# tarepan/DDSP-SVC-official

Hardware: AMD Instinct MI355X
Metric: audio samples/sec @44.1kHz CombSub synth (higher is better)
Workload: dtype f32 storage and accumulation; products of the GEMM / FIR contractions split-bf16x3 (hi*hi+hi*lo+lo*hi), of the attention split-bf16 from three pieces (6 products) for the feature projections and two (3 products) for the context sums; everything else f32; `value_fp32_mfma` is the leg with every produ; 1 GPU; CombSub 44.1 kHz, batch=64x2 s per GPU (Fr=172, T=88064), units/f0/volume/spk_id -> audio, seeded random weights, in-kernel noise

## Files before the change

### ddsp-svc-official_amd/csrc/gemm_f32.h

```cpp
#pragma once
#include "common.h"
#include "gemm_group.h"

#include <stdlib.h>
#include <type_traits>

namespace gemm {

enum { A_PLAIN = 0, A_CONV3 = 1, A_FRAMES = 2, A_CONVK = 3, A_DWCONV = 4 };

struct Args {
    const float* A;
    const float* B;
    int M, N, K;
    int64_t lda, ldb;
    int zdiv;
    int64_t sA_hi, sA_lo, sB_hi, sB_lo;
    int Fr, Cin;
    int tap_shift;
    int ktaps, dil;
    float in_slope;
    const float* zeros;
    int sub_from, parent_tn;
    int math;
    const float* B_split;
    int A_split;
    int xcd;
    int xcd_cut;
    int kz;
};

constexpr int BK = 32;
typedef float f32x4_u __attribute__((ext_vector_type(4), aligned(4)));

template <class E, class = void>
struct epi_wants_pair : std::false_type {};
template <class E>
struct epi_wants_pair<E, std::void_t<decltype(E::kPair)>> : std::true_type {};
template <class E, class = void>
struct epi_has_store4 : std::false_type {};
template <class E>
struct epi_has_store4<E, std::void_t<decltype(E::kStore4)>> : std::true_type {};
// ... 971 lines not shown
```

### ddsp-svc-official_amd/csrc/gemm_ln.h

```cpp
#pragma once
#include "gemm_f32.h"

#include <atomic>
#include <stdlib.h>

namespace gemm {

struct LnArgs {
    const float* A;
    const float* W;
    int64_t lda, ldw;
    int M, K;
    const float* bias;
    const float* res;
    float* X;
    const float* gamma;
    const float* beta;
    float* Y;
    int y_split;
    int Fr = 1, Cin = 32, tap_shift = 0;
    const float* zeros = nullptr;
    const float* dw_taps = nullptr;
    const float* dw_bias = nullptr;
    const int* n_frames = nullptr;
    int dw_left = 15;
};

struct PreResidual {
    struct State {
        f32x4 res[2][4];
        f32x4 bias4[4];
    };
    template <int RB>
    __device__ __forceinline__ void load(State& s, const LnArgs& g, int m0, int rg0, int lr, int cg, int lh) const {
#pragma unroll
        for (int b = 0; b < RB; ++b) {
            const int row_m = m0 + 32 * (rg0 + b) + lr;
#pragma unroll
            for (int q = 0; q < 4; ++q) {
                s.res[b][q] = f32x4{0.f, 0.f, 0.f, 0.f};
                if (row_m < g.M) s.res[b][q] = *(const f32x4*)(g.res + (int64_t)row_m * 256 + 32 * cg + 8 * q + 4 * lh);
            }
        }
#pragma unroll
        for (int q = 0; q < 4; ++q) s.bias4[q] = *(const f32x4*)(g.bias + 32 * cg + 8 * q + 4 * lh);
    }
    __device__ __forceinline__ f32x4 apply(const State& s, const LnArgs&, int b, int q, int, int, f32x4 acc) const {
        f32x4 v;
#pragma unroll
        for (int e = 0; e < 4; ++e) v[e] = s.res[b][q][e] + (acc[e] + s.bias4[q][e]);
        return v;
    }
};

constexpr int LN_BM = 64, LN_N = 256, LN_NS = 4;
constexpr int LN_STAGE = (LN_BM + LN_N) * 32;
constexpr size_t LN_LDS_BYTES = (size_t)LN_NS * LN_STAGE * sizeof(float);

constexpr int DWF_K = 31, DWF_C = 64, DWF_ROWS = LN_BM + DWF_K - 1, DWF_NSW = 3;
constexpr int DWF_W = LN_N * 32, DWF_IMG = LN_BM * 32;
constexpr int DWF_AIMG = DWF_NSW * DWF_W, DWF_RAW = DWF_AIMG + 4 * DWF_IMG, DWF_TAPS = DWF_RAW + 96 * DWF_C;
static_assert(DWF_TAPS + 32 * DWF_C == LN_NS * LN_STAGE, "the A_DWCONV layout fills the same LDS");

template <int NS, int RB, bool ASPLIT, int A_MODE, class Pre>
__global__ void __launch_bounds__(1024 / RB) kernel_res_ln(LnArgs g, Pre pre) {
    extern __shared__ __attribute__((aligned(1024))) float ln_lds[];
    float* const lds = ln_lds;
    constexpr int NWAVE = 16 / RB;
    const int tid = threadIdx.x, lane = tid & 63, wave = __builtin_amdgcn_readfirstlane(tid >> 6);
    const int rg0 = RB == 1 ? wave >> 3 : 0, cg = wave & 7, lr = lane & 31, lh = lane >> 5;
    const int nk = g.K / 32;
    int m0 = blockIdx.x * LN_BM;
    int dw_b = 0, dw_f0 = 0;
    if constexpr (A_MODE == A_DWCONV) {
        const int ftiles = (g.Fr + LN_BM - 1) / LN_BM;
        dw_b = blockIdx.x / ftiles;
        dw_f0 = (blockIdx.x % ftiles) * LN_BM;
        m0 = dw_b * g.Fr + dw_f0;
        g.M = dw_b * g.Fr + (dw_f0 + LN_BM < g.Fr ? dw_f0 + LN_BM : g.Fr);
    }

    typename Pre::State pst;
    pre.template load<RB>(pst, g, m0, rg0, lr, cg, lh);
    f32x4 gam4[4], bet4[4];
#pragma unroll
    for (int q = 0; q < 4; ++q) {
        const int c0 = 32 * cg + 8 * q + 4 * lh;
        gam4[q] = *(const f32x4*)(g.gamma + c0);
        bet4[q] = *(const f32x4*)(g.beta + c0);
    }
    static_assert(A_MODE == A_PLAIN || ((A_MODE == A_CONV3 || A_MODE == A_DWCONV) && RB == 2), "conv modes: eight waves, one A piece each");
    static_assert(A_MODE != A_DWCONV || ASPLIT, "the convolved operand is written in the split layout");

    typedef __bf16 bf16x8 __attribute__((ext_vector_type(8)));
    f32x16 acc[RB];
#pragma unroll
    for (int b = 0; b < RB; ++b)
#pragma unroll
        for (int r = 0; r < 16; ++r) acc[b][r] = 0.f;
    auto products = [&](const float* ast, const float* wst) {
        f32x4 xv[RB][4], wv[4];
#pragma unroll
        for (int b = 0; b < RB; ++b) {
            const int row = 32 * (rg0 + b) + lr;
            const float* rp = ast + row * 32;
#pragma unroll
            for (int c = 0; c < 4; ++c) xv[b][c] = *(const f32x4*)(rp + 4 * ((4 * lh + c) ^ ((row >> 1) & 7)));
        }
        {
            const int row = 32 * cg + lr;
            const float* rp = wst + row * 32;
#pragma unroll
            for (int c = 0; c < 4; ++c) wv[c] = *(const f32x4*)(rp + 4 * ((4 * lh + c) ^ ((row >> 1) & 7)));
        }
#pragma unroll
        for (int half = 0; half < 2; ++half) {
            const bf16x8 wh = __builtin_bit_cast(bf16x8, wv[2 * half]), wl = __builtin_bit_cast(bf16x8, wv[2 * half + 1]);
#pragma unroll
            for (int b = 0; b < RB; ++b) {
                bf16x8 xh, xl;
                if constexpr (ASPLIT) {
                    xh = __builtin_bit_cast(bf16x8, xv[b][2 * half]);
                    xl = __builtin_bit_cast(bf16x8, xv[b][2 * half + 1]);
                } else {
                    typedef float f32x2p __attribute__((ext_vector_type(2)));
                    typedef __bf16 bf16x2p __attribute__((ext_vector_type(2)));
                    ddsp_u32x4 wh_, wl_;
#pragma unroll
                    for (int d = 0; d < 4; ++d) {
                        const f32x4& src = d < 2 ? xv[b][2 * half] : xv[b][2 * half + 1];
                        f32x2p r = {src[(2 * d) & 3], src[(2 * d + 1) & 3]};
                        const uint32_t hh = __builtin_bit_cast(uint32_t, __builtin_convertvector(r, bf16x2p));
                        wh_[d] = hh;
                        r = r - (f32x2p){__builtin_bit_cast(float, hh << 16), __builtin_bit_cast(float, hh & 0xffff0000u)};
                        wl_[d] = __builtin_bit_cast(uint32_t, __builtin_convertvector(r, bf16x2p));
                    }
                    xh = __builtin_bit_cast(bf16x8, wh_);
                    xl = __builtin_bit_cast(bf16x8, wl_);
                }
                acc[b] = __builtin_amdgcn_mfma_f32_32x32x16_bf16(wh, xl, acc[b], 0, 0, 0);
                acc[b] = __builtin_amdgcn_mfma_f32_32x32x16_bf16(wl, xh, acc[b], 0, 0, 0);
                acc[b] = __builtin_amdgcn_mfma_f32_32x32x16_bf16(wh, xh, acc[b], 0, 0, 0);
            }
        }
    };

    if constexpr (A_MODE == A_DWCONV) {
        typedef float f32x2d __attribute__((ext_vector_type(2)));
        typedef __bf16 bf16x2d __attribute__((ext_vector_type(2)));
        float* const aimg = lds + DWF_AIMG;
        float* const raw = lds + DWF_RAW;
        float* const taps = lds + DWF_TAPS;
        const int nb = nk / 2;
        const int n_in = ddsp_row_frames(g.n_frames, dw_b, g.Fr);
        const int c4 = lane & 15;
        const float* rsrc[3];
        int radv[3];
#pragma unroll
        for (int i = 0; i < 3; ++i) {
            const int r = (wave + 8 * i) * 4 + (lane >> 4);
            const int f = dw_f0 + r - g.dw_left;
            const bool ok = r < DWF_ROWS && f >= 0 && f < n_in;
            rsrc[i] = ok ? g.A + ((int64_t)dw_b * g.Fr + f) * g.lda + 4 * c4 : g.zeros + 4 * c4;
            radv[i] = ok ? DWF_C : 0;
        }
        const int trow = 4 * wave + (lane >> 4);
        const float* const tsrc = trow < DWF_K ? g.dw_taps + (int64_t)trow * g.K + 4 * c4 : g.dw_bias + 4 * c4;
        const float* wsrc[4];
#pragma unroll
        for (int i = 0; i < 4; ++i) {
            const int n = (wave + 8 * i) * 8 + (lane >> 3);
            wsrc[i] = g.W + (int64_t)n * g.ldw + 4 * ((lane & 7) ^ ((n >> 1) & 7));
        }
        auto dma = [&](const float* p, float* dst) {
            __builtin_amdgcn_global_load_lds((const __attribute__((address_space(1))) void*)p,
                                             (__attribute__((address_space(3))) void*)dst, 16, 0, 0);
        };
        auto issue_raw = [&](int j) {
#pragma unroll
            for (int i = 0; i < 3; ++i) dma(rsrc[i] + j * radv[i], raw + (wave + 8 * i) * 256);
// ... 187 lines not shown
        for (int q = 0; q < 4; ++q) {
            const int c0 = 32 * cg + 8 * q + 4 * lh;
            f32x4 o;
#pragma unroll
            for (int e = 0; e < 4; ++e) o[e] = fmaf(d[b][q][e] * rs, gam4[q][e], bet4[q][e]);
            if (g.y_split) {
                const ddsp_u32x4 pk = ddsp_split4_pair(o, lh != 0, 32);
                if (row_ok) *(ddsp_u32x4*)(g.Y + (int64_t)row_m * LN_N + c0) = pk;
            } else if (row_ok)
                *(f32x4*)(g.Y + (int64_t)row_m * LN_N + c0) = o;
        }
    }
}

inline bool res_ln_ok(const LnArgs& g) {
    return g.K % 32 == 0 && g.K >= 64 && g.lda % 4 == 0 && g.ldw % 4 == 0 && g.M >= 1 &&
           (((uintptr_t)g.A | (uintptr_t)g.W | (uintptr_t)g.bias | (uintptr_t)g.res | (uintptr_t)g.X | (uintptr_t)g.gamma |
             (uintptr_t)g.beta | (uintptr_t)g.Y) % 16) == 0;
}

template <int RB, bool ASPLIT, int A_MODE = A_PLAIN, class Pre = PreResidual>
inline hipError_t launch_res_ln_rb(hipStream_t st, const LnArgs& g, const Pre& pre = Pre{}) {
    static std::atomic<uint64_t> done{0};
    int dev = 0;
    hipError_t e = hipGetDevice(&dev);
    if (e != hipSuccess) return e;
    const uint64_t bit = 1ull << (dev & 63);
    auto kfn = kernel_res_ln<LN_NS, RB, ASPLIT, A_MODE, Pre>;
    if (!(done.load(std::memory_order_acquire) & bit)) {
        e = hipFuncSetAttribute((const void*)kfn, hipFuncAttributeMaxDynamicSharedMemorySize, (int)LN_LDS_BYTES);
        if (e != hipSuccess) return e;
        done.fetch_or(bit, std::memory_order_release);
    }
    const int64_t tiles = A_MODE == A_DWCONV ? (int64_t)(g.M / g.Fr) * ((g.Fr + LN_BM - 1) / LN_BM) : (g.M + LN_BM - 1) / LN_BM;
    hipLaunchKernelGGL(kfn, dim3((unsigned)tiles), dim3(1024 / RB), LN_LDS_BYTES, st, g, pre);
    return hipSuccess;
}
inline hipError_t launch_res_ln(hipStream_t st, const LnArgs& g, bool a_split = true) {
    return a_split ? launch_res_ln_rb<2, true>(st, g) : launch_res_ln_rb<2, false>(st, g);
}

inline bool res_ln_dwconv_ok(const LnArgs& g) {
    return res_ln_ok(g) && g.K % 64 == 0 && g.Fr >= 1 && g.M % g.Fr == 0 && g.zeros && g.dw_taps && g.dw_bias && g.dw_left >= 0 &&
           g.dw_left < DWF_K && (((uintptr_t)g.zeros | (uintptr_t)g.dw_taps | (uintptr_t)g.dw_bias) % 16) == 0;
}
inline bool res_ln_dwconv_fills(int64_t B, int64_t Fr) {
    const int64_t own = B * ((Fr + LN_BM - 1) / LN_BM), rows = (B * Fr + LN_BM - 1) / LN_BM;
    return B >= 1 && Fr >= 1 && 4 * own <= 5 * rows;
}
inline hipError_t launch_res_ln_dwconv(hipStream_t st, const LnArgs& g) { return launch_res_ln_rb<2, true, A_DWCONV>(st, g); }

}
```

### ddsp-svc-official_amd/csrc/unit2ctrl_fwd.hip

```cpp
#include "gemm_f32.h"
#include "gemm_ws.h"
#include "gemm_ln.h"
#include "performer_attn.h"
#include "u2c.h"

using namespace u2c;

namespace {

__device__ __forceinline__ void store_group8(float* __restrict__ dst, const float (&x)[8], bool split) {
    if (split) {
        ddsp_u32x4 hi, lo;
        ddsp_split8(x, hi, lo);
        *(ddsp_u32x4*)dst = hi;
        *(ddsp_u32x4*)(dst + 4) = lo;
    } else {
        *(f32x4*)dst = f32x4{x[0], x[1], x[2], x[3]};
        *(f32x4*)(dst + 4) = f32x4{x[4], x[5], x[6], x[7]};
    }
}

__device__ __forceinline__ void pack_conv3_body(const float* __restrict__ w, int Cout, int Cin, float* __restrict__ out,
                                                int vb, int vgrid, bool split) {
    const int64_t groups = (int64_t)Cout * 3 * (Cin / 8);
// ... 325 lines not shown
            const int64_t id = spk_id[n_spk_id == 1 ? 0 : m / Fr];
            if (id >= 1 && id <= w.n_spk) {
                const v4 e = *(const v4*)(w.spk_table + (id - 1) * D + n);
#pragma unroll
                for (int j = 0; j < 4; ++j) v[j] += e[j];
            } else {
                __hip_atomic_store(err, DDSP_DEV_ERR_SPK_ID, __ATOMIC_RELAXED, __HIP_MEMORY_SCOPE_SYSTEM);
            }
        }
        return v;
    }
};

struct PreEmbed {
    EpiEmbed e;
    struct State {};
    template <int RB>
    __device__ __forceinline__ void load(State&, const gemm::LnArgs&, int, int, int, int, int) const {}
    __device__ __forceinline__ f32x4 apply(const State&, const gemm::LnArgs&, int, int, int m, int c0, f32x4 acc) const {
        return e.embed4(m, c0, acc);
    }
};

struct LnPending {
    const float* part;
    const float* bias;
    float* x_out;
    int has_res;
};
constexpr int KS_SPLITS = 4;
constexpr int KS_MAX_ROWS = 256;
constexpr int64_t U2C_PRESPLIT_MIN_ROWS = 8192;
constexpr int64_t U2C_DWCONV_FUSE_MIN_ROWS = 10240;
constexpr int64_t ATTN_BF16_MIN = 256;
__global__ void __launch_bounds__(256) layernorm_kernel(const float* __restrict__ x, const float* __restrict__ gamma,
                                                        const float* __restrict__ beta, int64_t rows,
                                                        float* __restrict__ out, int split, LnPending pend = LnPending{nullptr, nullptr, nullptr, 0}) {
    const int lane = threadIdx.x & 63;
    const int64_t m = (int64_t)blockIdx.x * 4 + (threadIdx.x >> 6);
    if (m >= rows) return;
    f32x4 v;
    if (pend.part) {
        const f32x4 p0 = *(const f32x4*)(pend.part + m * D + lane * 4), p1 = *(const f32x4*)(pend.part + (rows + m) * D + lane * 4);
        const f32x4 p2 = *(const f32x4*)(pend.part + (2 * rows + m) * D + lane * 4), p3 = *(const f32x4*)(pend.part + (3 * rows + m) * D + lane * 4);
        v = (p0 + p1) + (p2 + p3);
        if (pend.bias) v = v + *(const f32x4*)(pend.bias + lane * 4);
        if (pend.has_res) v = *(const f32x4*)(x + m * D + lane * 4) + v;
        *(f32x4*)(pend.x_out + m * D + lane * 4) = v;
    } else {
        v = *(const f32x4*)(x + m * D + lane * 4);
    }
    const float mean = wave_sum((v[0] + v[1]) + (v[2] + v[3])) * (1.0f / D);
    f32x4 d;
    float ss = 0.f;
#pragma unroll
    for (int j = 0; j < 4; ++j) {
        d[j] = v[j] - mean;
        ss = fmaf(d[j], d[j], ss);
    }
    const float rstd = 1.0f / sqrtf(wave_sum(ss) * (1.0f / D) + 1e-5f);
    const f32x4 ga = *(const f32x4*)(gamma + lane * 4), be = *(const f32x4*)(beta + lane * 4);
    f32x4 o;
#pragma unroll
    for (int j = 0; j < 4; ++j) o[j] = fmaf(d[j] * rstd, ga[j], be[j]);
    if (split)
        *(ddsp_u32x4*)(out + m * D + lane * 4) = ddsp_split4_pair(o, (lane & 1) != 0, 1);
// ... 426 lines not shown
        g.math = lin_math;
        if (presplit_w) {
            g.B = packed;
            g.B_split = packed;
            g.A_split = a_is_split;
        }
    };
    static const bool dw_tiled = [] { const char* e = getenv("DDSP_DW_PAIR"); return !(e && e[0] == '1'); }();
    bool conv_split = false;
    {
        gemm::Args g = gemm::make(in.units, w.n_unit, bf.w1, 3 * w.n_unit, iM, D, 3 * w.n_unit);
        set_b(g, bf.w1, 0);
        g.tap_shift = w.causal ? -1 : 0;
        g.Fr = (int)Fr;
        g.Cin = w.n_unit;
        g.zeros = zero_page;
        conv_split = ksplit && gemm::dma_ok(g) && g.K % (32 * KS_SPLITS) == 0 && w.n_unit % 32 == 0 && (3 * D) % (32 * KS_SPLITS) == 0 &&
                     w.n_unit + 32 <= DDSP_ZERO_FLOATS;
        if (conv_split) {
            g.K /= KS_SPLITS;
            g.kz = g.K;
            gemm::EpiStore e{bf.kpart, D, nullptr, 1, M * D, 0};
            PROF(PF_U2C_GEMM_CONV3, 2.0 * M * D * 3 * w.n_unit, 4.0 * M * (w.n_unit + D),
                 (gemm::dma_go<64, 64, gemm::EpiStore, 4, 4, gemm::A_CONV3>(st, g, KS_SPLITS, e)));
        } else {
            gemm::EpiStore e{bf.t1, D, w.prenet_conv1_b, 1, 0, 0};
            PROF(PF_U2C_GEMM_CONV3, 2.0 * M * D * 3 * w.n_unit, 4.0 * M * (w.n_unit + D),
                 (gemm::launch<true, true, gemm::A_CONV3>(st, g, 1, e)));
        }
    }
    PROF(PF_U2C_ROWWISE, 0, 4.0 * M * D,
         hipLaunchKernelGGL(groupnorm_stats_kernel, dim3(4, (unsigned)B), dim3(64 * GN_LANES), 0, st, bf.t1, (int)Fr, bf.gst,
                            conv_split ? bf.kpart : nullptr, w.prenet_conv1_b, M, in.n_frames));
    PROF(PF_U2C_ROWWISE, 0, 8.0 * M * D,
         hipLaunchKernelGGL(groupnorm_lrelu_kernel, dim3(grid_for(M * (D / 4))), dim3(256), 0, st, bf.t1, bf.gst,
                            w.prenet_gn_w, w.prenet_gn_b, M, (int)Fr, bf.t2, asplit, in.n_frames));
    float* x = bf.l[0].x_in;
    {
        gemm::Args g = gemm::make(bf.t2, D, bf.w2, 3 * D, iM, D, 3 * D);
        set_b(g, bf.w2, asplit);
        g.tap_shift = w.causal ? -1 : 0;
        g.Fr = (int)Fr;
        g.Cin = D;
        g.zeros = zero_page;
        if (conv_split) {
            g.K /= KS_SPLITS;
            g.kz = g.K;
            EpiEmbed e{bf.kpart, w.prenet_conv2_b, in.f0, in.phase, in.volume, w, in.spk_id, in.n_spk_id, in.mix, (int)Fr, dev_err, M * D};
            PROF(PF_U2C_GEMM_CONV3, 2.0 * M * D * 3 * D, 8.0 * M * D,
                 (gemm::dma_go<64, 64, EpiEmbed, 4, 4, gemm::A_CONV3>(st, g, KS_SPLITS, e)));
            pending = LnPending{bf.kpart, nullptr, x, 0};
        } else {
            EpiEmbed e{x, w.prenet_conv2_b, in.f0, in.phase, in.volume, w, in.spk_id, in.n_spk_id, in.mix, (int)Fr, dev_err, 0};
            gemm::LnArgs la = ln_args(g, x, x, w.prenet_conv2_b, w.layer[0].norm_w, w.layer[0].norm_b, bf.l[0].y);
            la.Fr = (int)Fr;
            la.Cin = D;
            la.tap_shift = g.tap_shift;
            la.zeros = zero_page;
            if (ln_fusable(g, la) && g.A_split && D + 32 <= DDSP_ZERO_FLOATS) {
                PROF(PF_U2C_GEMM_CONV3, 2.0 * M * D * 3 * D, 12.0 * M * D,
                     DDSP_HIP(ctx, (gemm::launch_res_ln_rb<2, true, gemm::A_CONV3, PreEmbed>(st, la, PreEmbed{e}))));
                ln_done = true;
            } else
                PROF(PF_U2C_GEMM_CONV3, 2.0 * M * D * 3 * D, 8.0 * M * D, (gemm::launch<true, true, gemm::A_CONV3>(st, g, 1, e)));
        }
    }
    DDSP_LAUNCH_CHECK(ctx);

    const unsigned rows_g = (unsigned)ceil_div64(M, 4), rows8_g = (unsigned)ceil_div64(M8, 4);
    auto feature_maps = [&](const LayerBufs& b, const float* proj) {
        gemm::Args g = gemm::make(b.q, DH, proj, DH, (int)M8, NF, DH);
// ... 270 lines not shown
extern "C" int ddsp_u2c_dwconv_pw2(ddsp_ctx* ctx, void* stream, const float* glu, const float* taps, const float* dw_bias,
                                   const float* W_split, const float* bias, const float* res, const float* gamma,
                                   const float* beta, const int* n_frames, int B, int Fr, int causal, int fused, float* scratch,
                                   float* X, float* Y) {
    DDSP_REQUIRE(ctx, ctx && glu && taps && dw_bias && W_split && bias && res && gamma && beta && X && Y && (fused || scratch),
                 "ddsp_u2c_dwconv_pw2: null argument");
    DDSP_REQUIRE(ctx, B >= 1 && Fr >= 1 && (int64_t)B * Fr < (1 << 26), "ddsp_u2c_dwconv_pw2: bad shape");
    const float* zero_page = nullptr;
    if (int rc = ddsp_zero_page(ctx, &zero_page)) return rc;
    hipStream_t st = (hipStream_t)stream;
    const int M = B * Fr, left = causal ? DWK - 1 : DWK / 2;
    gemm::LnArgs a{fused ? glu : scratch, W_split, INNER, INNER, M, INNER, bias, res, X, gamma, beta, Y, 1};
    a.Fr = Fr;
    a.zeros = zero_page;
    a.dw_taps = taps;
    a.dw_bias = dw_bias;
    a.n_frames = n_frames;
    a.dw_left = left;
    DDSP_REQUIRE(ctx, gemm::res_ln_dwconv_ok(a) && ((uintptr_t)glu % 16) == 0, "ddsp_u2c_dwconv_pw2: 16-byte aligned operands");
    DDSP_ENTER_DEVICE(ctx);
    ddsp_prof_begin(ctx, st, PF_OTHER);
    if (fused) {
        DDSP_HIP(ctx, gemm::launch_res_ln_dwconv(st, a));
    } else {
        hipLaunchKernelGGL(dwconv_tile_kernel, dim3(INNER / DWT_C, (unsigned)(B * ((Fr + DWT_F - 1) / DWT_F))), dim3(256), 0, st, glu,
                           taps, dw_bias, B, Fr, scratch, left, 1, n_frames);
        DDSP_HIP(ctx, gemm::launch_res_ln(st, a, true));
    }
    ddsp_prof_end(ctx, st, 2.0 * M * (double)D * INNER + 2.0 * M * (double)INNER * DWK, 4.0 * M * (INNER + 4.0 * D));
    DDSP_LAUNCH_CHECK(ctx);
    return DDSP_OK;
}

extern "C" int ddsp_unit2ctrl_fwd(ddsp_ctx* ctx, void* stream, const ddsp_u2c_weights* wp, const float* units,
                                  const float* f0_frames, const float* phase_frames, const float* volume,
                                  const int64_t* spk_id, int64_t n_spk_id, const int64_t* mix_ids_host,
                                  const float* mix_w_host, int n_mix, int64_t B, int64_t Fr, const int32_t* n_frames,
                                  float* ctrl) {
    return unit2ctrl_fwd_any(ctx, stream, wp, units, f0_frames, phase_frames, volume, spk_id, n_spk_id, mix_ids_host, mix_w_host,
                             n_mix, B, Fr, n_frames, ctrl);
}

extern "C" int ddsp_unit2ctrl_fwd_rowmix(ddsp_ctx* ctx, void* stream, const ddsp_u2c_weights* wp, const float* units,
                                         const float* f0_frames, const float* phase_frames, const float* volume,
                                         const int32_t* mix_ids_dev, const float* mix_w_dev, int K, int64_t B, int64_t Fr,
                                         const int32_t* n_frames, float* ctrl) {
    DDSP_REQUIRE(ctx, ctx && mix_ids_dev && mix_w_dev, "ddsp_unit2ctrl_fwd_rowmix: null mix table");
    DDSP_REQUIRE(ctx, K >= 1 && K <= 16, "ddsp_unit2ctrl_fwd_rowmix: 1 <= K <= 16 mixed speakers per row");
    const int64_t one_id = 1;
    const float zero_w = 0.f;
    return unit2ctrl_fwd_any(ctx, stream, wp, units, f0_frames, phase_frames, volume, nullptr, 0, &one_id, &zero_w, 1, B, Fr,
                             n_frames, ctrl, mix_ids_dev, mix_w_dev, K);
}

extern "C" int ddsp_unit2ctrl_fwd_framemix(ddsp_ctx* ctx, void* stream, const ddsp_u2c_weights* wp, const float* units,
                                           const float* f0_frames, const float* phase_frames, const float* volume,
                                           const int32_t* mix_ids_dev, const float* mix_w_dev, int K, int64_t B, int64_t Fr,
                                           const int32_t* n_frames, float* ctrl) {
    DDSP_REQUIRE(ctx, ctx && mix_ids_dev && mix_w_dev, "ddsp_unit2ctrl_fwd_framemix: null mix table");
    DDSP_REQUIRE(ctx, K >= 1 && K <= 16, "ddsp_unit2ctrl_fwd_framemix: 1 <= K <= 16 mixed speakers per frame");
    const int64_t one_id = 1;
    const float zero_w = 0.f;
    return unit2ctrl_fwd_any(ctx, stream, wp, units, f0_frames, phase_frames, volume, nullptr, 0, &one_id, &zero_w, 1, B, Fr,
                             n_frames, ctrl, mix_ids_dev, mix_w_dev, K, 1);
}

// ... 29 lines not shown
```

### ddsp-svc-official_amd/hipddsp/__init__.py

```python
import ctypes
import math as _math
import numbers
import os
import threading

import torch

_HERE = os.path.dirname(os.path.abspath(__file__))
LIB_PATH = os.path.join(_HERE, "libddsp_amd.so")

DDSP_OK, DDSP_ERR_ARG, DDSP_ERR_HIP, DDSP_ERR_OOM = 0, -1, -2, -3

COMB_NONE, COMB_SINC, COMB_SINC_GATED = 0, 1, 2
FIR_ALLPASS, FIR_DYNAMIC, FIR_STATIC = 0, 1, 2
EXC_AUDIO, EXC_UNIT_NOISE, EXC_GENERATE = 0, 1, 2
FIR_FP32, FIR_SPLIT_BF16 = 0, 3
ABI_VERSION = 8
MATH_FP32, MATH_SPLIT_BF16 = 0, 3
ATTENTION_CAUSAL = 200
SLICER_PAD = {"constant": 0, "reflect": 1}
ATTENTION_PAIR = 100

_c = ctypes
_vp, _i64, _u64, _int, _f32, _f64 = _c.c_void_p, _c.c_int64, _c.c_uint64, _c.c_int, _c.c_float, _c.c_double
# ... 114 lines not shown
    "ddsp_ctx_create": (_int, [_c.POINTER(_vp), _int]),
    "ddsp_ctx_destroy": (_int, [_vp]),
    "ddsp_last_error": (_c.c_char_p, [_vp]),
    "ddsp_ctx_reserve": (_int, [_vp, _u64]),
    "ddsp_ctx_poll_error": (_int, [_vp]),
    "ddsp_ctx_set_math": (_int, [_vp, _int]),
    "ddsp_ctx_get_math": (_int, [_vp]),
    "ddsp_upsample": (_int, [_vp, _vp, _vp, _i64, _i64, _i64, _int, _vp]),
    "ddsp_phase_scan": (_int, [_vp, _vp, _vp, _vp, _i64, _i64, _int, _int, _int, _int, _vp, _vp, _vp, _vp, _vp]),
    "ddsp_fir_from_ctrl": (_int, [_vp, _vp, _int, _vp, _i64, _int, _vp, _i64, _int, _vp]),
    "ddsp_fir_from_ctrl_group": (_int, [_vp, _vp, _vp, _i64, _i64, _int, _vp, _int]),
    "ddsp_ltv_fir_bwd": (_int, [_vp, _vp, _vp, _int, _u64, _vp, _vp, _i64, _i64, _int, _int, _vp, _vp]),
    "ddsp_fir_from_ctrl_bwd": (_int, [_vp, _vp, _int, _vp, _i64, _int, _vp, _i64, _int, _vp, _vp, _i64]),
    "ddsp_sins_bank": (_int, [_vp, _vp, _vp, _i64, _int, _vp, _vp, _i64, _i64, _int, _int, _vp]),
    "ddsp_spectral_ola": (_int, [_vp, _vp, _vp, _i64, _vp, _vp, _int, _u64, _i64, _i64, _int, _vp]),
    "ddsp_sins_bank_bwd": (_int, [_vp, _vp, _vp, _i64, _int, _vp, _vp, _vp, _i64, _i64, _int, _int, _vp, _i64]),
    "ddsp_spectral_ola_bwd": (_int, [_vp, _vp, _vp, _i64, _vp, _vp, _int, _u64, _vp, _i64, _i64, _int, _vp, _i64]),
    "ddsp_rss_loss": (_int, [_vp, _vp, _vp, _vp, _i64, _i64, _c.POINTER(_int), _vp, _c.POINTER(_int), _i64, _c.POINTER(_int),
                             _c.POINTER(_int), _int, _f32, _f32, _vp, _vp]),
    "ddsp_sola": (_int, [_vp, _vp, _vp, _int, _i64, _int, _int, _int, _int, _vp, _vp, _vp]),
    "ddsp_volume_gate": (_int, [_vp, _vp, _vp, _vp, _f32, _i64, _i64, _int]),
    "ddsp_volume_gate_rows": (_int, [_vp, _vp, _vp, _vp, _vp, _vp, _f32, _i64, _i64, _i64, _int]),
    "ddsp_volume_gate_files": (_int, [_vp, _vp, _vp, _vp, _vp, _i64, _vp, _vp, _vp, _f32, _i64, _i64, _i64, _int]),
    "ddsp_pieces_gather": (_int, [_vp] * 8 + [_i64, _i64, _i64, _vp, _i64, _i64, _i64, _vp, _vp, _vp]),
    "ddsp_pieces_gather_jobs": (_int, [_vp] * 8 + [_i64, _i64, _i64, _i64, _vp, _i64, _i64, _i64, _vp, _vp, _vp]),
    "ddsp_stitch": (_int, [_vp, _vp, _vp, _i64, _vp, _i64]),
    "ddsp_pcm16": (_int, [_vp, _vp, _vp, _i64, _vp, _i64, _vp, _vp, _vp]),
    "ddsp_phase_vocoder": (_int, [_vp, _vp, _vp, _vp, _vp, _vp, _int, _int, _vp]),
    "ddsp_volume_extract": (_int, [_vp, _vp, _vp, _i64, _i64, _vp, _int, _vp]),
    "ddsp_volume_extract_frac": (_int, [_vp, _vp, _vp, _i64, _i64, _f64, _vp]),
    "ddsp_align_units": (_int, [_vp, _vp, _vp, _i64, _i64, _i64, _i64, _f32, _vp, _vp, _vp]),
    "ddsp_gemm_res_ln": (_int, [_vp, _vp, _vp, _vp, _vp, _vp, _vp, _vp, _int, _int, _vp, _vp, _int]),
    "ddsp_u2c_dwconv_pw2": (_int, [_vp] * 11 + [_int, _int, _int, _int, _vp, _vp, _vp]),
    "ddsp_conv1d_pair_supported": (_int, [_vp, _int, _int, _int]),
    "ddsp_conv1d_pair": (_int, [_vp, _vp, _vp, _vp, _vp, _vp, _vp, _i64, _i64, _int, _int, _int, _f32, _vp, _vp, _vp, _int]),
    "ddsp_retime_f0": (_int, [_vp, _vp, _vp, _i64, _i64, _vp, _f64, _f64, _f32, _f64, _i64, _vp, _vp]),
    "ddsp_resample_length": (_i64, [_i64, _int, _int]),
    "ddsp_resample": (_int, [_vp, _vp, _vp, _i64, _i64, _vp, _int, _int, _int, _vp]),
    "ddsp_conv1d": (_int, [_vp, _vp, _vp, _vp, _vp, _i64, _i64, _int, _int, _int, _int, _f32, _vp, _vp, _vp, _f32, _vp, _int,
                           _vp, _int]),
    "ddsp_nsf_source": (_int, [_vp, _vp, _vp, _vp, _vp, _vp, _i64, _i64, _int, _int, _f32, _vp, _vp]),
    "ddsp_nsf_noise_conv": (_int, [_vp, _vp, _vp, _i64, _i64, _vp, _vp, _int, _int, _int, _int, _i64, _vp]),
    "ddsp_nsf_post": (_int, [_vp, _vp, _vp, _vp, _vp, _i64, _i64, _int, _int, _f32, _vp, _vp, _int]),
    "ddsp_nsf_mean": (_int, [_vp, _vp, _vp, _vp, _vp, _int, _i64, _vp, _vp, _f32, _int]),
    "ddsp_log_mel": (_int, [_vp, _vp, _vp, _vp, _vp, _i64, _int, _int, _f32, _vp]),
    "ddsp_adamw_step": (_int, [_vp, _vp, _vp, _vp, _vp, _vp, _i64, _f32, _f32, _f32, _f32, _f32, _i64]),
    "ddsp_adamw_step_multi": (_int, [_vp, _vp, _int, _vp, _vp, _vp, _vp, _vp, _f32, _f32, _f32, _f32, _f32, _i64, _f32]),
    "ddsp_gemm_f32": (_int, [_vp, _vp, _vp, _i64, _int, _vp, _i64, _int, _vp, _vp, _i64, _int, _int, _int, _int, _int]),
    "ddsp_performer_attention": (_int, [_vp, _vp, _vp, _vp, _vp, _vp, _i64, _i64, _vp, _int]),
    "ddsp_hubert_frames": (_i64, [_i64]),
    "ddsp_hubert_soft_units": (_int, [_vp, _vp, _c.POINTER(HubertWeights), _vp, _i64, _i64, _vp, _vp]),
    "ddsp_hubert_encode": (_int, [_vp, _vp, _c.POINTER(HubertWeights), _vp, _i64, _i64, _vp, _int, _vp]),
    "ddsp_softmax_attention": (_int, [_vp, _vp, _vp, _vp, _vp, _i64, _i64, _int, _vp, _int, _vp]),
    "ddsp_stft_frames": (_int, [_vp, _vp, _vp, _i64, _i64, _vp, _int, _int, _i64, _vp]),
    "ddsp_retime_f0_keyed": (_int, [_vp, _vp, _vp, _i64, _i64, _vp, _f64, _vp, _int, _vp, _vp, _f64, _i64, _vp, _vp]),
    "ddsp_enhancer_keys": (_int, [_vp, _vp, _vp, _i64, _i64, _i64, _int, _vp, _vp, _vp]),
    "ddsp_resample_keyed_plan": (_int, [_vp, _vp, _int, _c.POINTER(_int), _c.POINTER(_int), _int, _c.POINTER(_vp)]),
    "ddsp_resample_keyed_plan_destroy": (None, [_vp]),
    "ddsp_resample_keyed_length": (_i64, [_vp, _i64]),
    "ddsp_resample_keyed": (_int, [_vp, _vp, _vp, _vp, _i64, _i64, _vp, _vp, _vp]),
    "ddsp_crepe_frames": (_i64, [_i64, _int]),
    "ddsp_crepe_activations": (_int, [_vp, _vp, _c.POINTER(CrepeWeights), _vp, _i64, _i64, _vp, _vp, _i64, _int, _vp]),
    "ddsp_crepe_decode": (_int, [_vp, _vp, _vp, _i64, _i64, _vp, _f32, _f32, _i64, _u64, _vp, _int, _vp, _vp, _vp]),
    "ddsp_stream_push": (_int, [_vp, _vp, _vp, _int, _i64, _vp, _i64]),
    "ddsp_bank_gather": (_int, [_vp, _vp, _vp, _int, _int, _vp, _i64, _vp, _i64, _vp, _vp, _int, _vp, _vp, _vp, _int, _vp, _vp, _vp,
                                _vp, _vp, _vp]),
# ... 677 lines not shown
        Cout = w_packed.shape[0]
        if w_packed.shape[1] != ktaps * Cin:
            raise ValueError("conv1d: packed weight does not match (ktaps, Cin)")
        out = torch.empty(T, Cout, device=x.device, dtype=torch.float32) if want_out else None
        act = torch.empty(T, Cout, device=x.device, dtype=torch.float32) if act_slope is not None else None
        if out is None and act is None:
            raise ValueError("conv1d: nothing to return")
        flags = (CONV_X_SPLIT if x_split else 0) | (CONV_ACT_SPLIT if act_split else 0)
        B, Tr, n_dev, scale = self._rows("conv1d", rows, T)
        self.call("ddsp_conv1d", _ptr(x), _ptr(w_packed), _ptr(bias), B, Tr, Cin, Cout, int(ktaps), int(dil), float(in_slope),
                  _ptr(residual), _ptr(out), _ptr(act), float(act_slope if act_slope is not None else 1.0), _ptr(w_split), flags,
                  _ptr(n_dev), scale)
        return out if act_slope is None else (out, act)

    def gemm_res_ln(self, A_split, W_split, bias, res, gamma, beta, y_split=True, a_fp32=False):
        M, K = A_split.shape
        X = torch.empty(M, 256, device=A_split.device, dtype=torch.float32)
        Y = torch.empty(M, 256, device=A_split.device, dtype=torch.float32)
        self.call("ddsp_gemm_res_ln", _ptr(A_split), _ptr(W_split), _ptr(bias), _ptr(res), _ptr(gamma), _ptr(beta), int(M), int(K),
                  _ptr(X), _ptr(Y), (1 if y_split else 0) | (2 if a_fp32 else 0))
        return X, Y

    def u2c_dwconv_pw2(self, glu, taps, dw_bias, W_split, bias, res, gamma, beta, B, n_frames=None, causal=False, fused=True):
        M = glu.shape[0]
        if M % int(B):
            raise ValueError("u2c_dwconv_pw2: glu must hold B utterances of equal padded length")
        X = torch.empty(M, 256, device=glu.device, dtype=torch.float32)
        Y = torch.empty(M, 256, device=glu.device, dtype=torch.float32)
        scratch = None if fused else torch.empty(M, 512, device=glu.device, dtype=torch.float32)
        self.call("ddsp_u2c_dwconv_pw2", _ptr(glu), _ptr(taps), _ptr(dw_bias), _ptr(W_split), _ptr(bias), _ptr(res), _ptr(gamma),
                  _ptr(beta), _ptr(n_frames), int(B), M // int(B), 1 if causal else 0, 1 if fused else 0, _ptr(scratch), _ptr(X), _ptr(Y))
        return X, Y

    def conv1d_pair_supported(self, C, ktaps, dil):
        return bool(self.lib.ddsp_conv1d_pair_supported(self.handle, int(C), int(ktaps), int(dil)))

    def conv1d_pair(self, x, w1, b1, w2, b2, ktaps, dil, slope, want_out=True, want_act=False, rows=None):
        T, C = x.shape
        out = torch.empty(T, C, device=x.device, dtype=torch.float32) if want_out else None
        act = torch.empty(T, C, device=x.device, dtype=torch.float32) if want_act else None
        B, Tr, n_dev, scale = self._rows("conv1d_pair", rows, T)
        self.call("ddsp_conv1d_pair", _ptr(x), _ptr(w1), _ptr(b1), _ptr(w2), _ptr(b2), B, Tr, C, int(ktaps), int(dil), float(slope),
                  _ptr(out), _ptr(act), _ptr(n_dev), scale)
        return out, act

    def nsf_source(self, f0, rand_ini, lin_w, lin_b, upp, sr, sine_amp=0.1, n_dev=None):
        solo = f0.dim() == 1
        if solo and n_dev is not None:
            raise ValueError("nsf_source: n_dev needs f0 (B, L)")
        if not solo and tuple(rand_ini.shape) != (f0.shape[0], 9):
            raise ValueError(f"nsf_source: rand_ini must be (B, 9) = ({f0.shape[0]}, 9), got {tuple(rand_ini.shape)}")
        L = f0.shape[-1]
        rand_ini = rand_ini.contiguous().float()
        out = torch.empty(*f0.shape[:-1], L * int(upp), device=f0.device, dtype=torch.float32)
        self.call("ddsp_nsf_source", _ptr(f0), _ptr(rand_ini), _ptr(lin_w), _ptr(lin_b), 1 if solo else f0.shape[0], L, int(upp),
                  int(sr), float(sine_amp), _ptr(n_dev), _ptr(out))
        return out

    def nsf_noise_conv(self, src, w, b, K, stride, pad, T_out):
        B, T_src = (1, src.numel()) if src.dim() == 1 else src.shape
        C = w.shape[0]
        out = torch.empty(B * int(T_out), C, device=src.device, dtype=torch.float32)
        self.call("ddsp_nsf_noise_conv", _ptr(src), B, T_src, _ptr(w), _ptr(b), C, int(K), int(stride), int(pad), int(T_out), _ptr(out))
        return out

    def nsf_post(self, x, w, b, K, slope, rows=None):
# ... 618 lines not shown
```

### include/ddsp_amd.h

```cpp
#ifndef DDSP_AMD_H
#define DDSP_AMD_H

#include <stdint.h>

#ifdef __cplusplus
extern "C" {
#endif

#define DDSP_OK 0
#define DDSP_ERR_ARG (-1)
#define DDSP_ERR_HIP (-2)
#define DDSP_ERR_OOM (-3)

typedef struct ddsp_ctx ddsp_ctx;

int ddsp_ctx_create(ddsp_ctx** out, int device);
int ddsp_ctx_destroy(ddsp_ctx* ctx);
const char* ddsp_last_error(const ddsp_ctx* ctx);
int ddsp_ctx_reserve(ddsp_ctx* ctx, uint64_t bytes);
int ddsp_abi_version(void);
int ddsp_ctx_poll_error(ddsp_ctx* ctx);
#define DDSP_MATH_FP32 0
#define DDSP_MATH_SPLIT_BF16 3
int ddsp_ctx_set_math(ddsp_ctx* ctx, int math);
// ... 235 lines not shown
                     const int32_t* n_frames, int frame_scale);

int ddsp_nsf_source(ddsp_ctx* ctx, void* stream, const float* f0, const float* rand_ini, const float* lin_w,
                    const float* lin_b, int64_t B, int64_t L, int upp, int sr, float sine_amp, const int32_t* n_frames,
                    float* out);
int ddsp_nsf_noise_conv(ddsp_ctx* ctx, void* stream, const float* src, int64_t B, int64_t T_src, const float* w, const float* b,
                        int C, int K, int stride, int pad, int64_t T_out, float* out);
int ddsp_nsf_post(ddsp_ctx* ctx, void* stream, const float* x, const float* w, const float* b, int64_t B, int64_t T, int C, int K,
                  float slope, float* out, const int32_t* n_frames, int frame_scale);
int ddsp_nsf_mean(ddsp_ctx* ctx, void* stream, const float* a, const float* b, const float* c, int n_terms, int64_t n,
                  float* out, float* out_act, float act_slope, int flags);
int ddsp_log_mel(ddsp_ctx* ctx, void* stream, const float* frames, const float* dft_table, const float* mel_basis,
                 int64_t n_frames, int n_fft, int n_mels, float clip, float* out);
int ddsp_stft_frames(ddsp_ctx* ctx, void* stream, const float* audio, int64_t B, int64_t T, const int32_t* n_samples, int n_fft,
                     int hop, int64_t L, float* out);

int ddsp_adamw_step(ddsp_ctx* ctx, void* stream, float* param, const float* grad, float* exp_avg, float* exp_avg_sq,
                    int64_t n, float lr, float beta1, float beta2, float eps, float weight_decay, int64_t step);
int ddsp_adamw_step_multi(ddsp_ctx* ctx, void* stream, int n_tensors, float* const* params, const float* const* grads,
                          float* const* exp_avg, float* const* exp_avg_sq, const int64_t* numel, float lr,
                          float beta1, float beta2, float eps, float weight_decay, int64_t step, float grad_scale);

int ddsp_gemm_f32(ddsp_ctx* ctx, void* stream, const float* A, int64_t lda, int a_k_contig, const float* B,
                  int64_t ldb, int b_k_contig, const float* bias, float* C, int64_t ldc, int M, int N, int K, int tile,
                  int variant);

int ddsp_gemm_res_ln(ddsp_ctx* ctx, void* stream, const float* A_split, const float* W_split, const float* bias,
                     const float* res, const float* gamma, const float* beta, int M, int K, float* X, float* Y, int y_split);

int ddsp_u2c_dwconv_pw2(ddsp_ctx* ctx, void* stream, const float* glu, const float* taps, const float* dw_bias,
                        const float* W_split, const float* bias, const float* res, const float* gamma, const float* beta,
                        const int* n_frames, int B, int Fr, int causal, int fused, float* scratch, float* X, float* Y);

#define DDSP_ATTENTION_CAUSAL 200
#define DDSP_ATTENTION_PAIR 100
int ddsp_performer_attention(ddsp_ctx* ctx, void* stream, const float* q, const float* k, const float* v,
                             const float* proj, int64_t B, int64_t Fr, float* out, int math);

typedef struct ddsp_hubert_layer {
    const float *in_proj_w, *in_proj_b, *out_proj_w, *out_proj_b, *linear1_w, *linear1_b, *linear2_w, *linear2_b;
    const float *norm1_w, *norm1_b, *norm2_w, *norm2_b;
} ddsp_hubert_layer;

typedef struct ddsp_hubert_weights {
    const float *conv0_w, *norm0_w, *norm0_b;
    const float* conv_w[6];
    const float *fp_norm_w, *fp_norm_b, *fp_proj_w, *fp_proj_b;
    const float *pos_b, *pos_g, *pos_v;
    const float *norm_w, *norm_b;
    ddsp_hubert_layer layer[12];
    const float *proj_w, *proj_b;
    uint64_t version;
} ddsp_hubert_weights;

int64_t ddsp_hubert_frames(int64_t T);
int ddsp_hubert_soft_units(ddsp_ctx* ctx, void* stream, const ddsp_hubert_weights* w, const float* wav, int64_t B, int64_t T,
                           const int32_t* n_samples, float* units);
int ddsp_hubert_encode(ddsp_ctx* ctx, void* stream, const ddsp_hubert_weights* w, const float* wav, int64_t B, int64_t T,
                       const int32_t* n_samples, int layer, float* out);
int ddsp_softmax_attention(ddsp_ctx* ctx, void* stream, const float* q, const float* k, const float* v, int64_t B, int64_t L,
                           int heads, float* out, int math, const int32_t* n_keys);


typedef struct ddsp_crepe_weights {
    const float* conv_w[6];
    const float* conv_b[6];
// ... 47 lines not shown
```

Baseline: 5.419 billion samples/s.

## Fuse prenet GroupNorm+LeakyReLU into the conv2 residual-LayerNorm GEMM A-load

Adds an A_GNCONV3 mode to the residual-LayerNorm GEMM kernel. It loads the raw conv1 output tile, applies GroupNorm and LeakyReLU, and writes the split-bf16 hi/lo form into LDS once. The three conv taps then reuse that image by rotating row offsets, with halo rows patched in between taps. This removes the separate groupnorm_lrelu pass and its full activation round trip through global memory, at the cost of a more complex kernel with extra barriers. It only runs for large row counts when the other layout conditions hold. It also adds a standalone API entry point.

```diff
diff --git a/ddsp-svc-official_amd/csrc/gemm_f32.h b/ddsp-svc-official_amd/csrc/gemm_f32.h
--- a/ddsp-svc-official_amd/csrc/gemm_f32.h
+++ b/ddsp-svc-official_amd/csrc/gemm_f32.h
@@ -7,7 +7,7 @@
 
 namespace gemm {
 
-enum { A_PLAIN = 0, A_CONV3 = 1, A_FRAMES = 2, A_CONVK = 3, A_DWCONV = 4 };
+enum { A_PLAIN = 0, A_CONV3 = 1, A_FRAMES = 2, A_CONVK = 3, A_DWCONV = 4, A_GNCONV3 = 5 };
 
 struct Args {
     const float* A;
diff --git a/ddsp-svc-official_amd/csrc/gemm_ln.h b/ddsp-svc-official_amd/csrc/gemm_ln.h
--- a/ddsp-svc-official_amd/csrc/gemm_ln.h
+++ b/ddsp-svc-official_amd/csrc/gemm_ln.h
@@ -24,6 +24,9 @@
     const float* dw_bias = nullptr;
     const int* n_frames = nullptr;
     int dw_left = 15;
+    const float* gn_stats = nullptr;
+    const float* gn_gamma = nullptr;
+    const float* gn_beta = nullptr;
 };
 
 struct PreResidual {
@@ -61,6 +64,10 @@
 constexpr int DWF_W = LN_N * 32, DWF_IMG = LN_BM * 32;
 constexpr int DWF_AIMG = DWF_NSW * DWF_W, DWF_RAW = DWF_AIMG + 4 * DWF_IMG, DWF_TAPS = DWF_RAW + 96 * DWF_C;
 static_assert(DWF_TAPS + 32 * DWF_C == LN_NS * LN_STAGE, "the A_DWCONV layout fills the same LDS");
+
+constexpr int GNC_CIN = 256, GNC_CHUNKS = GNC_CIN / 32;
+constexpr int GNC_AIMG = DWF_NSW * DWF_W;
+static_assert(GNC_AIMG + GNC_CHUNKS * DWF_IMG == LN_NS * LN_STAGE, "the A_GNCONV3 layout fills the same LDS");
 
 template <int NS, int RB, bool ASPLIT, int A_MODE, class Pre>
 __global__ void __launch_bounds__(1024 / RB) kernel_res_ln(LnArgs g, Pre pre) {
@@ -72,7 +79,7 @@
     const int nk = g.K / 32;
     int m0 = blockIdx.x * LN_BM;
     int dw_b = 0, dw_f0 = 0;
-    if constexpr (A_MODE == A_DWCONV) {
+    if constexpr (A_MODE == A_DWCONV || A_MODE == A_GNCONV3) {
         const int ftiles = (g.Fr + LN_BM - 1) / LN_BM;
         dw_b = blockIdx.x / ftiles;
         dw_f0 = (blockIdx.x % ftiles) * LN_BM;
@@ -89,8 +96,9 @@
         gam4[q] = *(const f32x4*)(g.gamma + c0);
         bet4[q] = *(const f32x4*)(g.beta + c0);
     }
-    static_assert(A_MODE == A_PLAIN || ((A_MODE == A_CONV3 || A_MODE == A_DWCONV) && RB == 2), "conv modes: eight waves, one A piece each");
-    static_assert(A_MODE != A_DWCONV || ASPLIT, "the convolved operand is written in the split layout");
+    static_assert(A_MODE == A_PLAIN || ((A_MODE == A_CONV3 || A_MODE == A_DWCONV || A_MODE == A_GNCONV3) && RB == 2),
+                  "conv modes: eight waves, one A piece each");
+    static_assert((A_MODE != A_DWCONV && A_MODE != A_GNCONV3) || ASPLIT, "the operand formed here is written in the split layout");
 
     typedef __bf16 bf16x8 __attribute__((ext_vector_type(8)));
     f32x16 acc[RB];
@@ -98,11 +106,12 @@
     for (int b = 0; b < RB; ++b)
 #pragma unroll
         for (int r = 0; r < 16; ++r) acc[b][r] = 0.f;
-    auto products = [&](const float* ast, const float* wst) {
+    auto products = [&](const float* ast, const float* wst, int aoff = 0) {
         f32x4 xv[RB][4], wv[4];
 #pragma unroll
         for (int b = 0; b < RB; ++b) {
-            const int row = 32 * (rg0 + b) + lr;
+            int row = 32 * (rg0 + b) + lr;
+            if constexpr (A_MODE == A_GNCONV3) row = (row + aoff) & (LN_BM - 1);
             const float* rp = ast + row * 32;
 #pragma unroll
             for (int c = 0; c < 4; ++c) xv[b][c] = *(const f32x4*)(rp + 4 * ((4 * lh + c) ^ ((row >> 1) & 7)));
@@ -145,7 +154,111 @@
         }
     };
 
-    if constexpr (A_MODE == A_DWCONV) {
+    if constexpr (A_MODE == A_GNCONV3) {
+        float* const aimg = lds + GNC_AIMG;
+        const int kpt = nk / 3;
+        const int n_in = ddsp_row_frames(g.n_frames, dw_b, g.Fr);
+        auto dma = [&](const float* p, float* dst) {
+            __builtin_amdgcn_global_load_lds((const __attribute__((address_space(1))) void*)p,
+                                             (__attribute__((address_space(3))) void*)dst, 16, 0, 0);
+        };
+        const int oc = lane & 3, ch0 = 32 * wave + 8 * oc;
+        const f32x4 ga0 = *(const f32x4*)(g.gn_gamma + ch0), ga1 = *(const f32x4*)(g.gn_gamma + ch0 + 4);
+        const f32x4 be0 = *(const f32x4*)(g.gn_beta + ch0), be1 = *(const f32x4*)(g.gn_beta + ch0 + 4);
+        const float gmean = g.gn_stats[(dw_b * 4 + (wave >> 1)) * 2], grstd = g.gn_stats[(dw_b * 4 + (wave >> 1)) * 2 + 1];
+        auto frame_ok = [&](int i) {
+            const int f = dw_f0 + i - 1 + g.tap_shift;
+            return f >= 0 && f < n_in;
+        };
+        f32x4 late0 = {0.f, 0.f, 0.f, 0.f}, late1 = {0.f, 0.f, 0.f, 0.f};
+        const int late_i = LN_BM + ((lane >> 2) & 1);
+        const bool late_ok = lane < 8 && frame_ok(late_i);
+        if (late_ok) {
+            const float* p = g.A + ((int64_t)dw_b * g.Fr + (dw_f0 + late_i - 1 + g.tap_shift)) * g.lda + ch0;
+            late0 = *(const f32x4*)p;
+            late1 = *(const f32x4*)(p + 4);
+        }
+        {
+            const int r = 8 * wave + (lane >> 3);
+            const bool ok = frame_ok(r);
+            const int sl = (lane & 7) ^ ((r >> 1) & 7);
+            const float* src = ok ? g.A + ((int64_t)dw_b * g.Fr + (dw_f0 + r - 1 + g.tap_shift)) * g.lda + 4 * sl : g.zeros + 4 * sl;
+            const int adv = ok ? 32 : 0;
+#pragma unroll
+            for (int c = 0; c < GNC_CHUNKS; ++c) dma(src + c * adv, aimg + c * DWF_IMG + wave * 256);
+        }
+        const float* wsrc[4];
+#pragma unroll
+        for (int i = 0; i < 4; ++i) {
+            const int n = (wave + 8 * i) * 8 + (lane >> 3);
+            wsrc[i] = g.W + (int64_t)n * g.ldw + 4 * ((lane & 7) ^ ((n >> 1) & 7));
+        }
+        auto issue_w = [&](int kt) {
+            float* const st = lds + (kt % DWF_NSW) * DWF_W;
+#pragma unroll
+            for (int i = 0; i < 4; ++i) dma(wsrc[i] + kt * 32, st + (wave + 8 * i) * 256);
+        };
+        issue_w(0);
+        issue_w(1);
+        auto activate = [&](f32x4 v0, f32x4 v1, ddsp_u32x4& hi, ddsp_u32x4& lo) {
+            typedef float f32x2p __attribute__((ext_vector_type(2)));
+            typedef __bf16 bf16x2p __attribute__((ext_vector_type(2)));
+#pragma unroll
+            for (int d = 0; d < 4; ++d) {
+                f32x2p r;
+#pragma unroll
+                for (int e = 0; e < 2; ++e) {
+                    const int j = 2 * d + e;
+                    const float v = j < 4 ? v0[j & 3] : v1[j & 3];
+                    const float ga = j < 4 ? ga0[j & 3] : ga1[j & 3], be = j < 4 ? be0[j & 3] : be1[j & 3];
+                    const float y = fmaf((v - gmean) * grstd, ga, be);
+                    r[e] = y > 0.f ? y : 0.01f * y;
+                }
+                const uint32_t h = __builtin_bit_cast(uint32_t, __builtin_convertvector(r, bf16x2p));
+                hi[d] = h;
+                r = r - (f32x2p){__builtin_bit_cast(float, h << 16), __builtin_bit_cast(float, h & 0xffff0000u)};
+                lo[d] = __builtin_bit_cast(uint32_t, __builtin_convertvector(r, bf16x2p));
+            }
+        };
+        ddsp_u32x4 late_hi = {0u, 0u, 0u, 0u}, late_lo = {0u, 0u, 0u, 0u};
+        if (late_ok) activate(late0, late1, late_hi, late_lo);
+        asm volatile("s_waitcnt vmcnt(8)" ::: "memory");
+        __builtin_amdgcn_s_barrier();
+        {
+            float* const img = aimg + wave * DWF_IMG;
+#pragma unroll
+            for (int it = 0; it < 4; ++it) {
+                const int r = 16 * it + (lane >> 2), sw = (r >> 1) & 7;
+                if (frame_ok(r)) {
+                    float* const p0 = img + r * 32 + 4 * ((2 * oc) ^ sw);
+                    float* const p1 = img + r * 32 + 4 * ((2 * oc + 1) ^ sw);
+                    ddsp_u32x4 hi, lo;
+                    activate(*(const f32x4*)p0, *(const f32x4*)p1, hi, lo);
+                    *(ddsp_u32x4*)p0 = hi;
+                    *(ddsp_u32x4*)p1 = lo;
+                }
+            }
+        }
+        __syncthreads();
+        for (int kt = 0; kt < nk; ++kt) {
+            if (kt + 1 < nk)
+                asm volatile("s_waitcnt vmcnt(4)" ::: "memory");
+            else
+                asm volatile("s_waitcnt vmcnt(0)" ::: "memory");
+            __builtin_amdgcn_s_barrier();
+            if (kt + 2 < nk) issue_w(kt + 2);
+            const int tap = kt / kpt, c = kt - tap * kpt;
+            if (c == 0 && tap > 0) {
+                if (lane < 8 && (lane >> 2) == tap - 1) {
+                    float* const p = aimg + wave * DWF_IMG + (tap - 1) * 32 + 8 * oc;
+                    *(ddsp_u32x4*)p = late_hi;
+                    *(ddsp_u32x4*)(p + 4) = late_lo;
+                }
+                __syncthreads();
+            }
+            products(aimg + c * DWF_IMG, lds + (kt % DWF_NSW) * DWF_W, tap);
+        }
+    } else if constexpr (A_MODE == A_DWCONV) {
         typedef float f32x2d __attribute__((ext_vector_type(2)));
         typedef __bf16 bf16x2d __attribute__((ext_vector_type(2)));
         float* const aimg = lds + DWF_AIMG;
@@ -399,7 +512,7 @@
         if (e != hipSuccess) return e;
         done.fetch_or(bit, std::memory_order_release);
     }
-    const int64_t tiles = A_MODE == A_DWCONV ? (int64_t)(g.M / g.Fr) * ((g.Fr + LN_BM - 1) / LN_BM) : (g.M + LN_BM - 1) / LN_BM;
+    const int64_t tiles = (A_MODE == A_DWCONV || A_MODE == A_GNCONV3) ? (int64_t)(g.M / g.Fr) * ((g.Fr + LN_BM - 1) / LN_BM) : (g.M + LN_BM - 1) / LN_BM;
     hipLaunchKernelGGL(kfn, dim3((unsigned)tiles), dim3(1024 / RB), LN_LDS_BYTES, st, g, pre);
     return hipSuccess;
 }
@@ -417,4 +530,10 @@
 }
 inline hipError_t launch_res_ln_dwconv(hipStream_t st, const LnArgs& g) { return launch_res_ln_rb<2, true, A_DWCONV>(st, g); }
 
-}
+inline bool res_ln_gnconv3_ok(const LnArgs& g) {
+    return res_ln_ok(g) && g.Cin == GNC_CIN && g.K == 3 * GNC_CIN && g.lda == GNC_CIN && g.Fr >= 1 && g.M % g.Fr == 0 && g.zeros &&
+           g.gn_stats && g.gn_gamma && g.gn_beta && (g.tap_shift == 0 || g.tap_shift == -1) &&
+           (((uintptr_t)g.zeros | (uintptr_t)g.gn_gamma | (uintptr_t)g.gn_beta) % 16) == 0 && ((uintptr_t)g.gn_stats % 8) == 0;
+}
+
+}
diff --git a/ddsp-svc-official_amd/csrc/unit2ctrl_fwd.hip b/ddsp-svc-official_amd/csrc/unit2ctrl_fwd.hip
--- a/ddsp-svc-official_amd/csrc/unit2ctrl_fwd.hip
+++ b/ddsp-svc-official_amd/csrc/unit2ctrl_fwd.hip
@@ -381,6 +381,7 @@
 constexpr int KS_MAX_ROWS = 256;
 constexpr int64_t U2C_PRESPLIT_MIN_ROWS = 8192;
 constexpr int64_t U2C_DWCONV_FUSE_MIN_ROWS = 10240;
+constexpr int64_t U2C_GN_FUSE_MIN_ROWS = 10752;
 constexpr int64_t ATTN_BF16_MIN = 256;
 __global__ void __launch_bounds__(256) layernorm_kernel(const float* __restrict__ x, const float* __restrict__ gamma,
                                                         const float* __restrict__ beta, int64_t rows,
@@ -873,11 +874,34 @@
     PROF(PF_U2C_ROWWISE, 0, 4.0 * M * D,
          hipLaunchKernelGGL(groupnorm_stats_kernel, dim3(4, (unsigned)B), dim3(64 * GN_LANES), 0, st, bf.t1, (int)Fr, bf.gst,
                             conv_split ? bf.kpart : nullptr, w.prenet_conv1_b, M, in.n_frames));
-    PROF(PF_U2C_ROWWISE, 0, 8.0 * M * D,
-         hipLaunchKernelGGL(groupnorm_lrelu_kernel, dim3(grid_for(M * (D / 4))), dim3(256), 0, st, bf.t1, bf.gst,
-                            w.prenet_gn_w, w.prenet_gn_b, M, (int)Fr, bf.t2, asplit, in.n_frames));
     float* x = bf.l[0].x_in;
+    bool gn_fused = false;
     {
+        gemm::Args g = gemm::make(bf.t1, D, bf.w2, 3 * D, iM, D, 3 * D);
+        set_b(g, bf.w2, asplit);
+        gemm::LnArgs la = ln_args(g, x, x, w.prenet_conv2_b, w.layer[0].norm_w, w.layer[0].norm_b, bf.l[0].y);
+        la.Fr = (int)Fr;
+        la.Cin = D;
+        la.tap_shift = w.causal ? -1 : 0;
+        la.zeros = zero_page;
+        la.n_frames = in.n_frames;
+        la.gn_stats = bf.gst;
+        la.gn_gamma = w.prenet_gn_w;
+        la.gn_beta = w.prenet_gn_b;
+        gn_fused = asplit && !conv_split && M >= U2C_GN_FUSE_MIN_ROWS && ln_fusable(g, la) && gemm::res_ln_gnconv3_ok(la) &&
+                   gemm::res_ln_dwconv_fills(B, Fr);
+        if (gn_fused) {
+            EpiEmbed e{x, w.prenet_conv2_b, in.f0, in.phase, in.volume, w, in.spk_id, in.n_spk_id, in.mix, (int)Fr, dev_err, 0};
+            PROF(PF_U2C_GEMM_CONV3, 2.0 * M * D * 3 * D, 12.0 * M * D,
+                 DDSP_HIP(ctx, (gemm::launch_res_ln_rb<2, true, gemm::A_GNCONV3, PreEmbed>(st, la, PreEmbed{e}))));
+            ln_done = true;
+        }
+    }
+    if (!gn_fused)
+        PROF(PF_U2C_ROWWISE, 0, 8.0 * M * D,
+             hipLaunchKernelGGL(groupnorm_lrelu_kernel, dim3(grid_for(M * (D / 4))), dim3(256), 0, st, bf.t1, bf.gst,
+                                w.prenet_gn_w, w.prenet_gn_b, M, (int)Fr, bf.t2, asplit, in.n_frames));
+    if (!gn_fused) {
         gemm::Args g = gemm::make(bf.t2, D, bf.w2, 3 * D, iM, D, 3 * D);
         set_b(g, bf.w2, asplit);
         g.tap_shift = w.causal ? -1 : 0;
@@ -1214,6 +1238,45 @@
     return DDSP_OK;
 }
 
+extern "C" int ddsp_u2c_gn_conv2(ddsp_ctx* ctx, void* stream, const ddsp_u2c_weights* wp, const float* t1, const float* stats,
+                                 const float* W2_split, const float* f0, const float* phase, const float* volume,
+                                 const int64_t* spk_id, const int* n_frames, int B, int Fr, int fused, float* scratch, float* X,
+                                 float* Y) {
+    DDSP_REQUIRE(ctx, ctx && wp && t1 && stats && W2_split && f0 && phase && volume && spk_id && X && Y && (fused || scratch),
+                 "ddsp_u2c_gn_conv2: null argument");
+    DDSP_REQUIRE(ctx, B >= 1 && Fr >= 1 && (int64_t)B * Fr < (1 << 26), "ddsp_u2c_gn_conv2: bad shape");
+    const float* zero_page = nullptr;
+    if (int rc = ddsp_zero_page(ctx, &zero_page)) return rc;
+    int* dev_err = nullptr;
+    if (int rc = ddsp_dev_error_ptr(ctx, &dev_err)) return rc;
+    hipStream_t st = (hipStream_t)stream;
+    const ddsp_u2c_weights w = *wp;
+    const int M = B * Fr;
+    gemm::LnArgs a{fused ? t1 : scratch, W2_split, D, 3 * D, M, 3 * D, w.prenet_conv2_b, X, X, w.layer[0].norm_w, w.layer[0].norm_b, Y, 1};
+    a.Fr = Fr;
+    a.Cin = D;
+    a.tap_shift = w.causal ? -1 : 0;
+    a.zeros = zero_page;
+    a.n_frames = n_frames;
+    a.gn_stats = stats;
+    a.gn_gamma = w.prenet_gn_w;
+    a.gn_beta = w.prenet_gn_b;
+    DDSP_REQUIRE(ctx, gemm::res_ln_gnconv3_ok(a) && ((uintptr_t)t1 % 16) == 0, "ddsp_u2c_gn_conv2: 16-byte aligned operands");
+    DDSP_ENTER_DEVICE(ctx);
+    const PreEmbed pre{EpiEmbed{X, w.prenet_conv2_b, f0, phase, volume, w, spk_id, B, MixArgs{}, Fr, dev_err, 0}};
+    ddsp_prof_begin(ctx, st, PF_OTHER);
+    if (fused) {
+        DDSP_HIP(ctx, (gemm::launch_res_ln_rb<2, true, gemm::A_GNCONV3, PreEmbed>(st, a, pre)));
+    } else {
+        hipLaunchKernelGGL(groupnorm_lrelu_kernel, dim3(grid_for((int64_t)M * (D / 4))), dim3(256), 0, st, t1, stats, w.prenet_gn_w,
+                           w.prenet_gn_b, (int64_t)M, Fr, scratch, 1, n_frames);
+        DDSP_HIP(ctx, (gemm::launch_res_ln_rb<2, true, gemm::A_CONV3, PreEmbed>(st, a, pre)));
+    }
+    ddsp_prof_end(ctx, st, 2.0 * M * (double)D * 3 * D, 12.0 * M * (double)D);
+    DDSP_LAUNCH_CHECK(ctx);
+    return DDSP_OK;
+}
+
 extern "C" int ddsp_unit2ctrl_fwd(ddsp_ctx* ctx, void* stream, const ddsp_u2c_weights* wp, const float* units,
                                   const float* f0_frames, const float* phase_frames, const float* volume,
                                   const int64_t* spk_id, int64_t n_spk_id, const int64_t* mix_ids_host,
diff --git a/ddsp-svc-official_amd/hipddsp/__init__.py b/ddsp-svc-official_amd/hipddsp/__init__.py
--- a/ddsp-svc-official_amd/hipddsp/__init__.py
+++ b/ddsp-svc-official_amd/hipddsp/__init__.py
@@ -170,6 +170,7 @@
     "ddsp_align_units": (_int, [_vp, _vp, _vp, _i64, _i64, _i64, _i64, _f32, _vp, _vp, _vp]),
     "ddsp_gemm_res_ln": (_int, [_vp, _vp, _vp, _vp, _vp, _vp, _vp, _vp, _int, _int, _vp, _vp, _int]),
     "ddsp_u2c_dwconv_pw2": (_int, [_vp] * 11 + [_int, _int, _int, _int, _vp, _vp, _vp]),
+    "ddsp_u2c_gn_conv2": (_int, [_vp, _vp, _c.POINTER(U2CWeights)] + [_vp] * 8 + [_int, _int, _int, _vp, _vp, _vp]),
     "ddsp_conv1d_pair_supported": (_int, [_vp, _int, _int, _int]),
     "ddsp_conv1d_pair": (_int, [_vp, _vp, _vp, _vp, _vp, _vp, _vp, _i64, _i64, _int, _int, _int, _f32, _vp, _vp, _vp, _int]),
     "ddsp_retime_f0": (_int, [_vp, _vp, _vp, _i64, _i64, _vp, _f64, _f64, _f32, _f64, _i64, _vp, _vp]),
@@ -913,6 +914,17 @@
                   _ptr(beta), _ptr(n_frames), int(B), M // int(B), 1 if causal else 0, 1 if fused else 0, _ptr(scratch), _ptr(X), _ptr(Y))
         return X, Y
 
+    def u2c_gn_conv2(self, weights, t1, stats, W2_split, f0, phase, volume, spk_id, B, n_frames=None, fused=True):
+        M = t1.shape[0]
+        if M % int(B):
+            raise ValueError("u2c_gn_conv2: t1 must hold B utterances of equal padded length")
+        X = torch.empty(M, 256, device=t1.device, dtype=torch.float32)
+        Y = torch.empty(M, 256, device=t1.device, dtype=torch.float32)
+        scratch = None if fused else torch.empty(M, 256, device=t1.device, dtype=torch.float32)
+        self.call("ddsp_u2c_gn_conv2", ctypes.byref(weights), _ptr(t1), _ptr(stats), _ptr(W2_split), _ptr(f0), _ptr(phase),
+                  _ptr(volume), _ptr(spk_id), _ptr(n_frames), int(B), M // int(B), 1 if fused else 0, _ptr(scratch), _ptr(X), _ptr(Y))
+        return X, Y
+
     def conv1d_pair_supported(self, C, ktaps, dil):
         return bool(self.lib.ddsp_conv1d_pair_supported(self.handle, int(C), int(ktaps), int(dil)))
 
diff --git a/include/ddsp_amd.h b/include/ddsp_amd.h
--- a/include/ddsp_amd.h
+++ b/include/ddsp_amd.h
@@ -291,6 +291,10 @@
                         const float* W_split, const float* bias, const float* res, const float* gamma, const float* beta,
                         const int* n_frames, int B, int Fr, int causal, int fused, float* scratch, float* X, float* Y);
 
+int ddsp_u2c_gn_conv2(ddsp_ctx* ctx, void* stream, const ddsp_u2c_weights* w, const float* t1, const float* stats,
+                      const float* W2_split, const float* f0, const float* phase, const float* volume, const int64_t* spk_id,
+                      const int* n_frames, int B, int Fr, int fused, float* scratch, float* X, float* Y);
+
 #define DDSP_ATTENTION_CAUSAL 200
 #define DDSP_ATTENTION_PAIR 100
 int ddsp_performer_attention(ddsp_ctx* ctx, void* stream, const float* q, const float* k, const float* v,
```

Result: no change. 5.433 billion samples/s, median of 6 (+0.3%).
